# AlexanderGSC/gmres

Measured on AMD Instinct MI355X. Metric: Arnoldi iters/sec + HBM GB/s, 4096² Poisson-2D fp64, GMRES(m=95), higher is better.
Workload: dtype f64

## Files before the change

gmres_amd/_native.py:

```python
from __future__ import annotations

import ctypes
import os
import sys
import re

PKG = os.path.dirname(os.path.abspath(__file__))
LIB_DIR = os.environ.get("GK_LIB_DIR") or os.path.join(PKG, "lib")
HIP_SO = os.path.join(LIB_DIR, "libgmres_hip.so")
FHOST_SO = os.path.join(LIB_DIR, "libgmres_fhost.so")
HEADER = os.path.join(os.path.dirname(PKG), "include", "gmres_hip.h")

GK_OK = 0
GK_ERR_COMM = -6
GK_TUNE_PROJ_NT = 0
GK_TUNE_STENCIL_BLOCKS = 2
GK_TUNE_SR_BLOCKS = 28
GK_TUNE_SR_TWO_LEVEL = 29
GK_TUNE_XCHG_TIMEOUT_MS = 7
GK_TUNE_RES, GK_TUNE_RES_R2, GK_TUNE_RES_SHARE, GK_TUNE_RES_TIMEOUT_MS = 8, 9, 10, 11
GK_TUNE_VERR_ORDER = 14
GK_TUNE_HH_FUSE = 15
GK_TUNE_CHEB_STEN = 16
GK_TUNE_SPIN_WAIT = 18
GK_TUNE_GRAPH = 19
GK_TUNE_RES_QDEF = 20
GK_TUNE_RES_PC = 21
GK_TUNE_RES_FOLD = 22
GK_TUNE_RES_BLOCK = 23
GK_TUNE_WATCHDOG_MS = 24
GK_TUNE_HH_NORM_ORDER = 25
GK_TUNE_RES_PF = 27
GK_TUNE_RES_PIPE = 30
GK_TUNE_RIGHT_FUSED = 31
GK_SIDE_LEFT, GK_SIDE_RIGHT = 0, 1
GK_ERR_ARG, GK_ERR_STATE = -1, -4
GK_PREC_IDENTITY, GK_PREC_CBPR2, GK_PREC_CHEB = 0, 1, 2
(GK_KID_PROJ, GK_KID_STENCIL, GK_KID_SCALE, GK_KID_UPDATE, GK_KID_COMM, GK_KID_OTHER, GK_KID_RES, GK_KID_PREC,
 GK_KID_HALO, GK_KID_GRAPH) = range(10)
GK_KID_SR = 10
SR_PASS_NAMES = ["sr_cg_p", "sr_cg_x", "sr_cg_z", "sr_bi_p", "sr_bi_pc", "sr_bi_s", "sr_bi_sc", "sr_st1", "sr_st2",
                 "sr_bi_x", "sr_bi_pe", "sr_bi_se", "sr_dot", "sr_cg_xz", "sr_bi_pz", "sr_bi_sz"]
KID_NAMES = ["proj", "stencil", "scale", "update", "comm", "other", "res", "prec", "halo", "graph"] + SR_PASS_NAMES
GK_SR_PCG, GK_SR_BICGSTAB = 0, 1
COMM_KINDS = {0: None, 1: "rccl", 2: "local-group", 3: "xgmi-device-exchange"}
RES_VARIANTS = {0: None, 1: "prefetch", 2: "pairs", 3: "pairs+lds", 4: "w-only", 5: "w+column", 6: "blocked"}
RES_INFO_KEYS = ["variant", "G", "r2", "l2", "pf", "cw", "wo", "nt", "r2e", "l2e", "lds", "nres2", "pipe", "cheb_sten", "wt", "blk"]

c_int, c_double, c_ll, c_vp = ctypes.c_int, ctypes.c_double, ctypes.c_longlong, ctypes.c_void_p
_dp = ctypes.POINTER(ctypes.c_double)
_ip = ctypes.POINTER(ctypes.c_int)

_hip = None
_fhost = None


class GkError(RuntimeError):
    pass


def header_symbols() -> list[str]:
    txt = open(HEADER).read()
    return sorted(set(re.findall(r"^\s*(?:int|const char \*)\s*(gk_\w+)\s*\(", txt, re.M)))


_SIGS = {
    "gk_last_error": (ctypes.c_char_p, []),
    "gk_version": (c_int, []),
    "gk_runtime_info": (c_int, [_ip, _ip, _ip, ctypes.c_char_p, ctypes.c_char_p, c_int]),
    "gk_create": (c_int, [c_int, c_int, c_int, c_int, c_int, ctypes.POINTER(c_vp)]),
# ... 188 lines not shown
```

gmres_amd/csrc/gk_api.hip:

```cpp
#include <dlfcn.h>

#include <algorithm>
#include <cmath>
#include <cstdarg>
#include <cstdio>
#include <cstdlib>
#include <cstring>

#include "gk_blk.hpp"
#include "gk_host.hpp"
#include "gk_kernels.hpp"
#include "gk_resident.hpp"

using namespace gkh;
using gk::nt_auto_for;
using gk::plan_info;
using gk::plan_resident;
using gk::ResPlan;
using gk::RES_R2_BIG;

namespace gkh __attribute__((visibility("hidden"))) {

thread_local std::string g_err;

// ... 218 lines not shown

int fill_hash(gk_ctx *c, double *x, unsigned long long seed) {
    gk::k_fill_hash<<<c->nblk_stream, gk::TPB, 0, c->st>>>(x, c->nloc, c->g0, seed);
    LAUNCHCHK();
    return GK_OK;
}

int finalize(gk_ctx *c, const double *pin, int npin, double *out, int take_sqrt) {
    ProfScope ps(c, GK_KID_OTHER);
    gk::k_finalize<<<1, gk::TPB, 0, c->st>>>(pin, npin, out, take_sqrt);
    LAUNCHCHK();
    return GK_OK;
}

bool res_plan(gk_ctx *c, ResPlan &p, bool hh = false) {
    if (c->tune_res == 0 || c->res_broken || c->m > gk::RHMAX || c->res_cus <= 0 || c->res_gath == nullptr)
        return false;
    if (collective(c) && !(c->xs_on && c->nranks > 1)) return false;
    if (c->tune_res < 0 && c->res_share > 1) return false;
    const int gmax = std::max(1, std::min(gk::RGMAX, c->res_cus / std::max(1, c->res_share)));
    const int cap = c->tune_res_r2 > 0 ? c->tune_res_r2 : RES_R2_BIG;
    plan_resident(c->nloc, gmax, cap, c->tune_res_wonly, hh,
                  c->tune_nt > 0 || (c->tune_nt < 0 && c->nt_auto), p, c->tune_res_pc, c->tune_res_blk, c->tune_res_pf,
                  c->tune_res_pipe);
    if (p.wo && !hh && c->m + 1 > gk::WO_HMAX) return false;
    return true;
}

enum { RESF_CLOSE_HH = 1, RESF_UNIT_INIT = 2, RESF_PIN_LOCAL = 4 };
int res_step(gk_ctx *c, int j, const ResPlan &p, const double *pin, int npin, double *hs, double *hcopy,
             int mode = gk::RES_MGS, double *w = nullptr, i64 unit_g = -1, int flags = 0) {
    ProfScope ps(c, GK_KID_RES);
    const bool close = (flags & RESF_CLOSE_HH) && mode == gk::RES_HH_UP;
    if ((flags & ~RESF_PIN_LOCAL) != 0 && !p.wo)
        return set_err(GK_ERR_STATE, "resident flags %d need the w-only variant", flags);
    const bool pin_local = (flags & RESF_PIN_LOCAL) && mode != gk::RES_HH_DOWN && c->xs_on && c->nranks > 1;
    const int np = (mode == gk::RES_MGS ? (p.bvar >= 0 ? gk::blk_exchanges(j, p.blk) : 2 * j) : j) + (close ? 1 : 0);
    if (c->res_tag > 0xF0000000u) {
        HIPCHK(hipMemsetAsync(c->res_gath, 0, sizeof(gk::u64) * gk::RES_GATH_ALL, c->st));
        c->res_tag = 1;
    }
    gk::ResArgs a{};
    a.w = w != nullptr ? w : c->w;
    a.mode = mode;
    a.coef = mode == gk::RES_MGS ? 1.0 : 2.0;
    a.tail0 = mode == gk::RES_HH_UP ? (i64)j - c->g0 : 0;
    a.V = c->V;
// ... 1134 lines not shown
int gk_set_tuning(gk_ctx *c, int key, int value) {
    CHK(check_ctx(c));
    switch (key) {
        case GK_TUNE_PROJ_NT: c->tune_nt = value < 0 ? -1 : (value != 0); break;
        case GK_TUNE_PROJ_BLOCKS: c->tune_pj_blocks = value; break;
        case GK_TUNE_STENCIL_BLOCKS: c->tune_st_blocks = value; break;
        case GK_TUNE_CHEB_FUSED: c->tune_cheb_fused = value != 0; break;
        case GK_TUNE_XCHG_TIMEOUT_MS:
            if (value < 1) return set_err(GK_ERR_ARG, "timeout must be >= 1 ms");
            xs_set_timeout(c, value);
            break;
        case GK_TUNE_RES: c->tune_res = value < 0 ? -1 : (value != 0); break;
        case GK_TUNE_RES_R2:
            if (value != 0 && value != 2 && value != 4 && value != 8 && value != 12)
                return set_err(GK_ERR_ARG, "resident cap must be 0 (auto), 2, 4, 8 or 12");
            c->tune_res_r2 = value;
            break;
        case GK_TUNE_RES_SHARE:
            if (value < 1) return set_err(GK_ERR_ARG, "share must be >= 1");
            c->res_share = value;
            break;
        case GK_TUNE_RES_WONLY: c->tune_res_wonly = value < 0 ? -1 : (value != 0); break;
        case GK_TUNE_RES_PIPE: c->tune_res_pipe = value < 0 ? -1 : (value != 0); break;
        case GK_TUNE_HH_FUSE: c->tune_hh_fuse = value != 0; break;
        case GK_TUNE_CHEB_STEN: c->tune_cheb_sten = value != 0; break;
        case GK_TUNE_SPIN_WAIT: c->tune_spin_wait = value != 0; break;
        case GK_TUNE_GRAPH: c->tune_graph = value != 0; break;
        case GK_TUNE_RES_QDEF: c->tune_res_qdef = value < 0 ? -1 : (value != 0); break;
        case GK_TUNE_RES_PC: c->tune_res_pc = value < 0 ? -1 : (value != 0); break;
        case GK_TUNE_RES_FOLD: c->tune_res_fold = value != 0; break;
        case GK_TUNE_WATCHDOG_MS: c->watchdog_ms = std::max(0, value); break;
        case GK_TUNE_HH_NORM_ORDER: c->tune_hh_norm_order = value != 0; break;
        case GK_TUNE_RES_BLOCK:
            if (value != 1 && value != 2 && value != 4)
                return set_err(GK_ERR_ARG, "GK_TUNE_RES_BLOCK %d: blocks of 1 (strict MGS-R), 2 or 4 projections", value);
            if (c->cycle_mgs)
                c->pend_res_blk = value;
            else
                c->tune_res_blk = value;
            break;
        case GK_TUNE_SR_BLOCKS: c->tune_sr_blocks = std::max(0, value); break;
        case GK_TUNE_SR_TWO_LEVEL: c->tune_sr_two = value != 0; break;
        case GK_TUNE_RES_PF:
            if (c->cycle_mgs)
                c->pend_res_pf = value != 0;
            else
// ... 460 lines not shown
```

gmres_amd/csrc/gk_host.hpp:

```cpp
#pragma once
#include <hip/hip_runtime.h>
#include <rccl/rccl.h>

#include <condition_variable>
#include <deque>
#include <mutex>
#include <string>
#include <vector>

#include "../../include/gmres_hip.h"
#include "gk_res.hpp"

using gk::i64;

namespace gk {
struct SrDev;
struct SrMirror;
}

struct gk_group {
    int n = 0;
    std::mutex mu;
    std::condition_variable cv;
    int arrived = 0;
// ... 41 lines not shown
    i64 xs_words = 0;
    gk::XsPeers xs_peers{};
    std::vector<void *> xs_mapped;
    bool xs_ready = false, xs_on = false, xs_broken = false;
    unsigned xs_seq = 0, xs_hseq = 0;
    int *xs_err = nullptr, *xs_err_dev = nullptr;
    long long xs_tick_per_ms = 100000;
    int xs_timeout_ms = 20000;
    gk::u64 xs_timeout = 0;
    gk::u64 *res_gath = nullptr;
    double *res_gm = nullptr;
    int tune_res_blk = 1;
    int tune_res_pf = 0;
    int pend_res_blk = 0, pend_res_pf = -1;
    int watchdog_ms = 0;
    bool broken = false;
    unsigned *hold_word = nullptr, *hold_word_dev = nullptr;
    int *res_err = nullptr, *res_err_dev = nullptr;
    unsigned res_tag = 1;
    int res_cus = 0;
    int tune_res = -1;
    int tune_res_r2 = 0;
    int tune_res_pipe = -1;
    int tune_res_wonly = -1;
    int tune_verr_order = 1;
    int tune_hh_fuse = 1;
    int tune_hh_norm_order = 0;
    int res_share = 1;
    int res_timeout_ms = 20000;
    bool res_broken = false;
    gk::u64 *res_stamps = nullptr;
    bool res_split = false;
    gk::u64 *res_trace = nullptr;
    int res_trace_j = 0, res_trace_mode = -1;
    int res_trace_g = 0, res_trace_np = 0;
    int vec = 2, JT = 16;
    dim3 sgrid;
    int sr_JT = 64, tune_sr_blocks = 0;
    int tune_sr_two = 1;
    bool sr_two = false;
    dim3 sr_sgrid;
    int np_sr = 0;
    int np_st = 0, np_pj = 0, nblk_stream = 0;
    int last_np = 0;
    int tune_cheb_fused = 1;
    int tune_cheb_sten = 1;
// ... 103 lines not shown
```

gmres_amd/csrc/gk_res.hpp:

```cpp
#pragma once
#include "gk_common.hpp"
#include "gk_cheb.hpp"

namespace gk {

constexpr int XS_MAXR = 16;
constexpr int XS_MAXV = 128;
constexpr i64 XS_RED_WORDS = 2LL * XS_MAXR * XS_MAXV * 2;
typedef unsigned long long u64;
struct XsPeers {
    u64 *p[XS_MAXR];
};
enum { XS_SLAB = 0, XS_VEC = 1, XS_BCAST = 2 };

__device__ __forceinline__ void xs_put(u64 *q, unsigned seq, unsigned data) {
    __hip_atomic_store(q, ((u64)seq << 32) | data, __ATOMIC_RELAXED, __HIP_MEMORY_SCOPE_SYSTEM);
}

__device__ __forceinline__ int xs_flag(const int *err) {
    return __hip_atomic_load(err, __ATOMIC_RELAXED, __HIP_MEMORY_SCOPE_SYSTEM);
}

enum { XG_ABORT = -1, XG_LATE = 0, XG_OK = 1 };
__device__ __forceinline__ int xs_get(const u64 *q, unsigned seq, u64 deadline, unsigned *data, const int *err) {
// ... 174 lines not shown
    for (int q = 0; q < a.nranks; ++q) {
        const unsigned lo = __shfl(d, 2 * q, 64), hi = __shfl(d, 2 * q + 1, 64);
        const double v = __longlong_as_double((long long)(((u64)hi << 32) | lo));
        r = (q == 0) ? v : r + v;
    }
    return r;
}

__device__ __forceinline__ bool res_pin_fold(const ResArgs &a, double &h, double *bc, int *okf) {
    if (!a.pin_local) return true;
    if (threadIdx.x < 64) {
        bool ok = true;
        const double r = res_rank_sum(a, -1, h, ok);
        if (threadIdx.x == 0) {
            bc[0] = r;
            *okf = ok ? 1 : 0;
        }
    }
    __syncthreads();
    h = bc[0];
    return *okf != 0;
}

template <int NW = RWAVES, bool TR = false, int SLEEP = RES_POLL_SLEEP>
__device__ __forceinline__ void res_exchange(const ResArgs &a, int p, const double *sm, double *bc, int *okf) {
    const int lane = threadIdx.x;
    const int G = gridDim.x;
    const unsigned tag = a.tag0 + (unsigned)p;
    auto rep_slot = [&](int r) -> u64 * {
        return a.gath + (RES_NREP > 1 ? RES_REP0 + r * RES_REP_STRIDE : 0) + (i64)(p & 1) * G * 2;
    };
    u64 *slot = rep_slot((int)(blockIdx.x % RES_NREP));
    double s = sm[0];
#pragma unroll
    for (int w = 1; w < NW; ++w) s += sm[w];
    u64 t_pub = 0;
    if (TR && a.trace != nullptr) t_pub = wall_clock64();
    if (RES_PUSHERS > 1 && res_pusher(a)) asm volatile("s_waitcnt vmcnt(0)" ::: "memory");
    if (lane < 2 * RES_NREP) {
        const u64 bits = (u64)__double_as_longlong(s);
        const int half = lane & 1;
        __hip_atomic_store(rep_slot(lane >> 1) + 2 * blockIdx.x + half,
                           ((u64)tag << 32) | (half ? (unsigned)(bits >> 32) : (unsigned)bits), __ATOMIC_RELAXED,
                           __HIP_MEMORY_SCOPE_AGENT);
    }
    const u64 deadline = wall_clock64() + a.timeout;
    double acc = 0.0;
    bool all_ok = true;
    if (a.nranks == 1 || blockIdx.x < RES_PUSHERS) {
        for (int c0 = 0; c0 < 2 * G && all_ok; c0 += 512) {
            unsigned v[8];
            for (;;) {
                u64 x[8];
#pragma unroll
                for (int k = 0; k < 8; ++k) {
                    const int g = c0 + lane + 64 * k;
                    x[k] = __hip_atomic_load(slot + (g < 2 * G ? g : 0), __ATOMIC_RELAXED, __HIP_MEMORY_SCOPE_AGENT);
                }
                bool ok = true;
#pragma unroll
                for (int k = 0; k < 8; ++k) {
                    const bool in = c0 + lane + 64 * k < 2 * G;
                    v[k] = in ? (unsigned)x[k] : 0u;
                    ok = ok && (!in || (unsigned)(x[k] >> 32) == tag);
                }
                if (__all(ok)) break;
                if (wall_clock64() > deadline) {
                    all_ok = false;
// ... 119 lines not shown
```

gmres_amd/csrc/gk_resident.hip:

```cpp
#include <hip/hip_runtime.h>

#include <algorithm>
#include <atomic>
#include <cstdarg>
#include <cstdio>

#include "../../include/gmres_hip.h"
#include "gk_blk.hpp"
#include "gk_res.hpp"
#include "gk_resident.hpp"

namespace gk {

template <int R2, int L2, bool PF, bool NT, bool CW, int MODE>
__global__ __launch_bounds__(RT, 2) void k_mgs_res(ResArgs a) {
    extern __shared__ double2 lw[];
    __shared__ double sm[RWAVES];
    __shared__ double bc[1];
    __shared__ int okf;
    __shared__ double hsh[RHMAX + 1];
    constexpr int RB = PF ? R2 : 1;
    constexpr int DT = CW ? RT - 64 : RT;
    const int t = threadIdx.x;
    const bool data = !CW || t >= 64;
// ... 264 lines not shown
#define GK_RES_TOUCH 24
#endif
constexpr int TOUCH = GK_RES_TOUCH;
#ifndef GK_RES_TOUCH_MGS
#define GK_RES_TOUCH_MGS 28
#endif
constexpr int TOUCH_MGS = GK_RES_TOUCH_MGS;
#ifndef GK_RES_TOUCH_MGS_PIPE
#define GK_RES_TOUCH_MGS_PIPE 20
#endif
constexpr int TOUCH_MGS_PIPE = GK_RES_TOUCH_MGS_PIPE;
#ifndef GK_RES_TOUCH_PACE
#define GK_RES_TOUCH_PACE 24
#endif
constexpr int TOUCH_PACE = GK_RES_TOUCH_PACE;
#ifndef GK_RES_TOUCH_PACE_HH
#define GK_RES_TOUCH_PACE_HH 0
#endif
constexpr int TOUCH_PACE_HH = GK_RES_TOUCH_PACE_HH;
#ifndef GK_RES_PIPE_D
#define GK_RES_PIPE_D 8
#endif
constexpr int PIPE_D = GK_RES_PIPE_D;

template <class F, int... I>
__device__ __forceinline__ void seq_apply(F &&f, std::integer_sequence<int, I...>) {
    (f(std::integral_constant<int, I>{}), ...);
}
template <int N, class F>
__device__ __forceinline__ void seq_for(F &&f) {
    seq_apply(f, std::make_integer_sequence<int, N>{});
}

template <int RW, int LW, int MODE, int WBT = WB, bool PIPE = false>
__global__ __launch_bounds__(WT, 1) void k_mgs_wres(ResArgs a) {
    extern __shared__ double2 lw[];
    __shared__ double sm[WT / 64];
    __shared__ double bc[1];
    __shared__ int okf;
    __shared__ int xdone;
    __shared__ double hsh[MODE == RES_MGS ? WO_HMAX : 1];
    const int t = threadIdx.x;
    constexpr int mode = MODE;
    constexpr int PACE = MODE == RES_MGS ? TOUCH_PACE : TOUCH_PACE_HH;
    constexpr int TCH = MODE == RES_MGS ? (PIPE ? TOUCH_MGS_PIPE : TOUCH_MGS) : TOUCH;
    const int j = a.j, np = res_np(mode, j);
    const i64 n2 = a.n >> 1, ld2 = a.ld >> 1;
    const i64 nch = a.nres2 / WT;
    const i64 bq = blockIdx.x;
    const i64 c0 = bq * a.r2e, cend = c0 + a.r2e < nch ? c0 + a.r2e : nch;
    const i64 l0 = (i64)gridDim.x * a.r2e + bq * a.l2e, lend = l0 + a.l2e < nch ? l0 + a.l2e : nch;
    const i64 tail0 = mode == RES_HH_UP ? a.tail0 : 0;
    const double2 *__restrict__ V2 = reinterpret_cast<const double2 *>(a.V);
    double2 *__restrict__ W2 = reinterpret_cast<double2 *>(a.w);
    ResClock clk;
    clk.start(a.stamps);
    int touch_sink = 0;
    const i64 sstride = (i64)gridDim.x * WT;
    const i64 sbase = a.nres2 + (i64)res_stream_wg() * WT + t;
    double2 wr[RW];
    if (mode == RES_HH_DOWN && a.unit_init) {
        const i64 u = a.unit_e;
        auto unit2 = [&](i64 e2) { return double2{2 * e2 == u ? 1.0 : 0.0, 2 * e2 + 1 == u ? 1.0 : 0.0}; };
#pragma unroll
        for (int k = 0; k < RW; ++k) wr[k] = (c0 + k < cend) ? unit2((c0 + k) * WT + t) : double2{0.0, 0.0};
        for (int k = 0; k < LW; ++k)
            if (l0 + k < lend) lw[k * WT + t] = unit2((l0 + k) * WT + t);
        for (i64 e = sbase; e < n2; e += sstride) W2[e] = unit2(e);
        if ((a.n & 1) && blockIdx.x == gridDim.x - 1 && t == 0) a.w[a.n - 1] = (a.n - 1 == u) ? 1.0 : 0.0;
    } else {
#pragma unroll
        for (int k = 0; k < RW; ++k) wr[k] = (PIPE || c0 + k < cend) ? W2[(c0 + k) * WT + t] : double2{0.0, 0.0};
        for (int k = 0; k < LW; ++k)
            if (PIPE || l0 + k < lend) lw[k * WT + t] = W2[(l0 + k) * WT + t];
    }
    auto red = [&](double &acc, const double2 &v, const double2 &b, int kind, i64 e2, bool chk) {
        if (kind == RK_DOT) {
            acc = acc + v.x * b.x;
            acc = acc + v.y * b.y;
        } else if (kind == RK_NORM) {
            sq_acc(acc, v, e2, tail0, chk);
        }
    };
    const i64 wc0 = c0, wl0 = l0;
    auto pass = [&](double ch, int i, int q, int kind) -> double {
        const double2 *__restrict__ A2 = V2 + (i64)i * ld2;
        const double2 *__restrict__ B2 = V2 + (i64)q * ld2;
        const bool dot = kind == RK_DOT;
        double acc = 0.0;
        i64 c0 = wc0, l0 = wl0;
        if constexpr (PIPE) {
            int zero = 0;
            asm volatile("" : "+s"(zero));
            c0 += zero;
            l0 += zero;
        }
        if constexpr (PIPE) {
            constexpr int D = WBT, NCH = RW + LW;
            static_assert(MODE == RES_MGS && NCH > D && 2 * (D - 1) <= 63,
                          "pipelined pass: the MGS step, counts within vmcnt's 6 bits, V_q default policy");
            d2v pa[D], pb[D];
            const unsigned lo = (unsigned)t * (unsigned)sizeof(double2);
            const double2 *Ar = A2 + c0 * WT, *Al = A2 + l0 * WT, *Br = B2 + c0 * WT, *Bl = B2 + l0 * WT;
            __builtin_amdgcn_s_waitcnt(0x0f70);
            auto held = [&](int k) { return k < RW ? c0 + k < cend : l0 + (k - RW) < lend; };
            auto issue = [&](auto kc) {
                constexpr int k = decltype(kc)::value;
                const double2 *ap = k < RW ? Ar + k * WT : Al + (k - RW) * WT;
                const double2 *bq = k < RW ? Br + k * WT : Bl + (k - RW) * WT;
                const double2 *bp = dot ? bq : Ar;
                d2v &da = pa[k % D], &db = pb[k % D];
                const unsigned off = lo;
                asm volatile("global_load_dwordx4 %0, %1, %2 nt" : "=v"(da) : "v"(off), "s"(ap));
                asm volatile("global_load_dwordx4 %0, %1, %2" : "=v"(db) : "v"(off), "s"(bp));
            };
            auto wait = [&](auto kc) {
                constexpr int k = decltype(kc)::value;
                constexpr int younger = NCH - 1 - k < D - 1 ? NCH - 1 - k : D - 1;
                d2v &da = pa[k % D], &db = pb[k % D];
                asm volatile("s_waitcnt vmcnt(%2)" : "+v"(da), "+v"(db) : "i"(2 * younger));
            };
            auto consume = [&](auto kc) {
                constexpr int k = decltype(kc)::value;
                const double2 av{pa[k % D].x, pa[k % D].y}, bv{pb[k % D].x, pb[k % D].y};
                if (!held(k)) return;
                if constexpr (k < RW) {
                    wr[k].x = wr[k].x - ch * av.x;
                    wr[k].y = wr[k].y - ch * av.y;
                    red(acc, wr[k], bv, kind, (c0 + k) * WT + t, false);
                } else {
                    constexpr int kl = k - RW;
                    double2 wv = lw[kl * WT + t];
                    wv.x = wv.x - ch * av.x;
                    wv.y = wv.y - ch * av.y;
                    lw[kl * WT + t] = wv;
                    red(acc, wv, bv, kind, (l0 + kl) * WT + t, false);
                }
            };
            seq_for<D>(issue);
            seq_for<NCH>([&](auto kc) {
                constexpr int k = decltype(kc)::value;
                wait(kc);
                consume(kc);
                if constexpr (k + D < NCH) issue(std::integral_constant<int, k + D>{});
            });
            return acc;
        }
        auto rbatch = [&](const int k0) {
            double2 av[WBT], bv[WBT];
#pragma unroll
            for (int u = 0; u < WBT; ++u) {
                const i64 c = c0 + k0 + u;
                if (k0 + u < RW && c < cend) {
                    av[u] = ldv<true>(A2 + c * WT + t);
                    if (dot) bv[u] = ldv<false>(B2 + c * WT + t);
                }
            }
#pragma unroll
            for (int u = 0; u < WBT; ++u) {
                const int k = k0 + u;
                if (k < RW && c0 + k < cend) {
                    wr[k].x = wr[k].x - ch * av[u].x;
// ... 38 lines not shown
                    if (dot) bv[u] = ldv<false>(B2 + e);
                }
            }
#pragma unroll
            for (int u = 0; u < 2; ++u) {
                const i64 e = e0 + u * sstride;
                if (e < n2) {
                    wv[u].x = wv[u].x - ch * av[u].x;
                    wv[u].y = wv[u].y - ch * av[u].y;
                    W2[e] = wv[u];
                    red(acc, wv[u], bv[u], kind, e, mode == RES_HH_UP && 2 * a.nres2 < tail0);
                }
            }
        }
        if ((a.n & 1) && blockIdx.x == gridDim.x - 1 && t == 0) {
            const i64 e = a.n - 1;
            const double x = a.w[e] - ch * a.V[(i64)i * a.ld + e];
            a.w[e] = x;
            if (kind == RK_DOT) acc = acc + x * a.V[(i64)q * a.ld + e];
            if (kind == RK_NORM && e >= tail0) acc = acc + x * x;
        }
        return acc;
    };
    int xi = 0;
    auto reduce = [&](double acc, double &h, int touch_col) -> bool {
        clk.passed(a.stamps);
        acc = wave_sum(acc);
        if ((t & 63) == 0) sm[t >> 6] = acc;
        if (PACE > 0 && t == 0) xdone = 0;
        __syncthreads();
        if (t < 64) {
            res_exchange<WT / 64, MODE == RES_MGS, RES_POLL_SLEEP>(a, xi, sm, bc, &okf);
            if (PACE > 0 && t == 0) *(volatile int *)&xdone = 1;
        } else if constexpr (TCH > 0) {
            if (touch_col >= 0) {
                const i64 r0 = c0, r1 = cend;
                const i64 lines = (i64)32 * (r1 - r0 < TCH ? (r1 - r0 > 0 ? r1 - r0 : 0) : TCH);
                const char *base = reinterpret_cast<const char *>(V2 + (i64)touch_col * ld2 + r0 * WT);
                for (i64 l = t - 64; l < lines; l += WT - 64) {
                    if constexpr (PACE > 0) {
                        if (*(volatile int *)&xdone) break;
                    }
                    const char *ptr = base + l * 128;
                    asm volatile("global_load_dword %0, %1, off" : "+v"(touch_sink) : "v"(ptr) : "memory");
                    if constexpr (PACE > 0) __builtin_amdgcn_s_sleep(PACE);
                }
            }
        }
        __syncthreads();
        if constexpr (TCH > 0) asm volatile("s_waitcnt vmcnt(0)" : : "v"(touch_sink) : "memory");
        ++xi;
        h = bc[0];
        clk.waited(a.stamps);
        return okf != 0;
    };
    auto kind_of = [&](int p) { return p < np - 1 ? RK_DOT : (mode == RES_MGS ? RK_NORM : RK_NONE); };
    double h;
    bool ok = true;
    if (mode == RES_HH_DOWN) {
        const int q = res_col(mode, j, 0);
        double acc = 0.0;
        if (a.unit_known) {
            if (blockIdx.x == 0 && t == 0 && a.unit_e >= 0) acc = a.V[(i64)q * a.ld + a.unit_e];
        } else {
            acc = pass(0.0, q, q, RK_DOT);
        }
        ok = reduce(acc, h, kind_of(0) == RK_DOT ? res_col(mode, j, 1) : -1);
    } else {
        double s = 0.0;
        for (int k = t; k < a.npin; k += WT) s += a.pin[k];
        s = wave_sum(s);
        if ((t & 63) == 0) sm[t >> 6] = s;
        __syncthreads();
        h = sm[0];
#pragma unroll
        for (int w = 1; w < WT / 64; ++w) h += sm[w];
        __syncthreads();
        ok = res_pin_fold(a, h, bc, &okf);
    }
    for (int p = 0; p < np && ok; ++p) {
        const int i = res_col(mode, j, p);
        const int kind = kind_of(p);
        if (mode == RES_MGS && blockIdx.x == 0 && t == 0) hsh[i] = (p < j ? 0.0 : hsh[i]) + h;
        const double acc = pass(mode == RES_MGS ? h : a.coef * h, i, res_col(mode, j, p + 1), kind);
        if (kind != RK_NONE)
            ok = reduce(acc, h, p + 1 < np && kind_of(p + 1) == RK_DOT ? res_col(mode, j, p + 2) : -1);
    }
    if (!ok) return;
    const bool close = mode == RES_HH_UP && a.close_hh;
    if (mode != RES_MGS) {
        double acc = 0.0;
        const bool up = mode == RES_HH_UP;
#pragma unroll
        for (int k = 0; k < RW; ++k)
            if (c0 + k < cend) {
                if (!close) W2[(c0 + k) * WT + t] = wr[k];
                if (up) sq_acc(acc, wr[k], (c0 + k) * WT + t, tail0, c0 + k == 0);
            }
        for (int k = 0; k < LW; ++k)
            if (l0 + k < lend) {
                const double2 v = lw[k * WT + t];
                if (!close) W2[(l0 + k) * WT + t] = v;
                if (up) sq_acc(acc, v, (l0 + k) * WT + t, tail0, l0 + k == 0);
            }
        if (up) {
            for (i64 e = sbase; e < n2; e += sstride) sq_acc(acc, W2[e], e, tail0, 2 * e < tail0 + 2);
            if ((a.n & 1) && blockIdx.x == gridDim.x - 1 && t == 0 && a.n - 1 >= tail0) {
                const double x = a.w[a.n - 1];
                acc = acc + x * x;
// ... 332 lines not shown
    if (RES_PCS && n2 <= (i64)G * RES_PCS_RW * RES_PC_NT) return 8 * n2;
    const int rx = hh ? RES_PC_RX : RES_PC_RX_MGS;
    const i64 cap = (i64)G * RES_PC_RW * RES_PC_NT, cached = (i64)G * (rx + RES_PC_LX) * RES_PC_NT;
    const i64 r = std::min(n2, cap), c = std::min(r, cached);
    return 8 * c + 16 * (r - c) + 32 * (n2 - r);
}

i64 pairs_bytes(i64 n2, int G) {
    const i64 rp = (i64)G * RES_R2_BIG * gk::RT, lp = (i64)G * RES_L2 * gk::RT;
    auto clamp = [](i64 v) { return v < 0 ? (i64)0 : v; };
    const i64 pr = std::min(n2, rp), pl = std::min(clamp(n2 - rp), lp), ps = clamp(n2 - rp - lp);
    return 8 * pr + 16 * pl + 32 * ps;
}

i64 wonly_bytes(i64 n2, int G) {
    const i64 rw = (i64)G * (RES_RW + RES_LW) * gk::WT;
    const i64 wr = std::min(n2, rw), ws = n2 > rw ? n2 - rw : 0;
    return 16 * wr + 32 * ws;
}

static bool wonly_pays(i64 n2, int G) { return wonly_bytes(n2, G) < pairs_bytes(n2, G); }

void plan_resident(i64 nloc, int gmax, int cap, int tune_wonly, bool hh, bool nt, ResPlan &p,
                   int tune_pc, int tune_blk, int tune_pf, int tune_pipe) {
    const i64 n2 = nloc / 2;
    const i64 dcw = gk::RT - 64;
    const int gcw = (int)std::max<i64>(1, std::min<i64>(gmax, (n2 + 2 * dcw - 1) / (2 * dcw)));
    const i64 need = (n2 + (i64)gcw * dcw - 1) / ((i64)gcw * dcw);
    p = ResPlan{};
    static const int pfs[] = {2, 4, 8};
    for (int s : pfs)
        if (s <= cap && (p.r2 == 0 || p.r2 < need)) p.r2 = s;
    auto spread = [&](i64 dt, int rmax, int lmax) {
        const i64 nchf = n2 / dt, G = p.G;
        p.r2e = (int)std::min<i64>(rmax, (nchf + G - 1) / G);
        const i64 rest = std::max<i64>(0, nchf - G * p.r2e);
        p.l2e = (int)std::min<i64>(lmax, (rest + G - 1) / G);
        p.nres2 = std::min<i64>(nchf, G * (p.r2e + p.l2e)) * dt;
    };
    const int var = gk::blk_variant((n2 + (i64)gmax * 512 - 1) / ((i64)gmax * 512));
    const bool pf = !hh && tune_blk == 1 && var != gk::BLK_WONLY && tune_pf > 0;
    if (!hh && (tune_blk > 1 || pf)) {
        p.G = gmax;
        const gk::BlkGeom g = gk::blk_geom(var, tune_blk);
        p.blk = tune_blk;
        p.bvar = var;
        p.wt = g.nt;
// ... 12 lines not shown
        p.pf = p.cw = true;
        spread(dcw, p.r2, 0);
    } else if (tune_wonly <= 0 && (tune_pc > 0 ? pc_fits : (tune_pc < 0 && pc_pays))) {
        p.G = gmax;
        p.pc = true;
        p.wt = RES_PC_NT;
        spread(RES_PC_NT, RES_PC_RW, 0);
        p.pcs = RES_PCS && p.r2e <= RES_PCS_RW;
        p.r2 = p.pcs ? RES_PCS_RX : (hh ? RES_PC_RX : RES_PC_RX_MGS);
        p.l2 = p.pcs ? RES_PCS_LX : RES_PC_LX;
        p.lds = p.l2 * RES_PC_NT * (int)sizeof(double2);
        p.nt = true;
        return;
    } else if (tune_wonly > 0 || (tune_wonly < 0 && wonly_pays(n2, gmax))) {
        p.G = gmax;
        p.wo = true;
        p.wt = gk::WT;
        p.r2 = 0;
        spread(gk::WT, hh ? RES_RW_HH : RES_RW, hh ? RES_LW_HH : RES_LW);
        p.lds = (hh ? RES_LW_HH : RES_LW) * gk::WT * (int)sizeof(double2);
        p.nt = true;
        p.pipe = RES_PIPE_OK && !hh && (tune_pipe < 0 ? RES_PIPE : tune_pipe != 0) && p.r2e == RES_RW &&
                 p.l2e == RES_LW && nloc % 2 == 0 && n2 == (i64)p.G * (RES_RW + RES_LW) * gk::WT && p.nres2 == n2;
        return;
    } else {
        p.G = gmax;
        p.r2 = RES_R2_BIG;
        const i64 dt = gk::RT, regs = (i64)p.G * RES_R2_BIG * dt;
        p.l2 = n2 / dt * dt > regs ? RES_L2 : 0;
        spread(dt, RES_R2_BIG, p.l2);
    }
    p.lds = std::max<int>(RES_LDS_MIN, p.l2 * (p.cw ? gk::RT - 64 : gk::RT) * (int)sizeof(double2));
    p.wt = gk::RT;
    p.nt = nt;
}

bool nt_auto_for(i64 max_nloc) { return max_nloc * 8 > (i64)48 * 1024 * 1024; }

void plan_info(const ResPlan &p, bool on, long long *info) {
    for (int k = 0; k < GK_RES_INFO_LEN; ++k) info[k] = 0;
    if (!on) return;
    info[RPI_VARIANT] = p.bvar >= 0 ? GK_RES_BLOCKED
                        : p.pc    ? GK_RES_WCOL
                                  : (p.wo ? GK_RES_WONLY
                                          : (p.pf ? GK_RES_PREFETCH : (p.l2 > 0 ? GK_RES_PAIRS_LDS : GK_RES_PAIRS)));
    info[RPI_BLK] = p.bvar >= 0 ? p.blk : 1;
    info[RPI_G] = p.G;
    info[RPI_R2] = p.r2;
    info[RPI_L2] = p.l2;
    info[RPI_PF] = p.pf;
    info[RPI_CW] = p.cw;
    info[RPI_WO] = p.wo;
    info[RPI_NT] = p.nt;
    info[RPI_R2E] = p.r2e;
    info[RPI_L2E] = p.l2e;
    info[RPI_LDS] = p.lds;
    info[RPI_NRES2] = p.nres2;
    info[RPI_WT] = p.wt;
    info[RPI_PIPE] = p.pipe;
}

namespace {

int fail(std::string &msg, int code, const char *fmt, ...) {
    char buf[512];
    va_list ap;
    va_start(ap, fmt);
    vsnprintf(buf, sizeof buf, fmt, ap);
    va_end(ap);
    msg = buf;
    return code;
}

int dyn_lds(const void *kernel, int dev, int lds, std::atomic<int> *memo, std::string &msg) {
    if (dev < 0 || dev >= ATTR_DEVS) return fail(msg, GK_ERR_ARG, "device id %d out of range", dev);
    const hipError_t e = ensure_dyn_lds(kernel, dev, lds, memo);
    if (e != hipSuccess)
        return fail(msg, GK_ERR_HIP, "%s:%d hipFuncSetAttribute(dynamic LDS %d): %s", __FILE__, __LINE__, lds,
                    hipGetErrorString(e));
    return GK_OK;
}

// ... 1 lines not shown
    const hipError_t e = hipGetLastError();
    if (e != hipSuccess) return fail(msg, GK_ERR_HIP, "resident step launch: %s", hipGetErrorString(e));
    return GK_OK;
}

template <int R2, int L2, bool PF, bool NT, bool CW, int MODE>
int launch_res_m(const ResPlan &p, const ResArgs &a, int dev, hipStream_t st, std::string &msg) {
    static std::atomic<int> attr[ATTR_DEVS];
    const int e = dyn_lds(reinterpret_cast<const void *>(&k_mgs_res<R2, L2, PF, NT, CW, MODE>), dev, p.lds, attr, msg);
    if (e != GK_OK) return e;
    k_mgs_res<R2, L2, PF, NT, CW, MODE><<<p.G, RT, p.lds, st>>>(a);
    return launched(msg);
}

template <int R2, int L2, bool PF, bool NT, bool CW>
int launch_res_t(const ResPlan &p, const ResArgs &a, int dev, hipStream_t st, std::string &msg) {
    switch (a.mode) {
        case RES_HH_UP: return launch_res_m<R2, L2, PF, NT, CW, RES_HH_UP>(p, a, dev, st, msg);
        case RES_HH_DOWN: return launch_res_m<R2, L2, PF, NT, CW, RES_HH_DOWN>(p, a, dev, st, msg);
        default: return launch_res_m<R2, L2, PF, NT, CW, RES_MGS>(p, a, dev, st, msg);
    }
}

template <int MODE, bool PIPE = false>
int launch_wres_m(const ResPlan &p, const ResArgs &a, int dev, hipStream_t st, std::string &msg) {
    constexpr int RW = MODE == RES_MGS ? RES_RW : RES_RW_HH;
    constexpr int LW = MODE == RES_MGS ? RES_LW : RES_LW_HH;
    constexpr int WBT = PIPE ? PIPE_D : (MODE == RES_MGS ? WB : WB_HH);
    static std::atomic<int> attr[ATTR_DEVS];
    const int e = dyn_lds(reinterpret_cast<const void *>(&k_mgs_wres<RW, LW, MODE, WBT, PIPE>), dev, p.lds, attr, msg);
    if (e != GK_OK) return e;
    k_mgs_wres<RW, LW, MODE, WBT, PIPE><<<p.G, WT, p.lds, st>>>(a);
    return launched(msg);
}

int launch_wres(const ResPlan &p, const ResArgs &a, int dev, hipStream_t st, std::string &msg) {
    switch (a.mode) {
        case RES_HH_UP: return launch_wres_m<RES_HH_UP>(p, a, dev, st, msg);
        case RES_HH_DOWN: return launch_wres_m<RES_HH_DOWN>(p, a, dev, st, msg);
        default:
            if constexpr (RES_PIPE_OK) {
                if (p.pipe) {
                    if (p.r2e != RES_RW || p.l2e != RES_LW || (a.n & 1) || a.nres2 != a.n / 2)
                        return fail(msg, GK_ERR_STATE, "pipelined w-only step on a plan that is not full (%d + %d chunks)",
                                    p.r2e, p.l2e);
                    return launch_wres_m<RES_MGS, true>(p, a, dev, st, msg);
                }
            }
            return launch_wres_m<RES_MGS>(p, a, dev, st, msg);
    }
}

template <int RW, int RX, int LX, int MODE>
int launch_wpc_k(const ResPlan &p, const ResArgs &a, int dev, hipStream_t st, std::string &msg) {
    constexpr int WBT = MODE == RES_MGS ? RES_PC_WB : RES_PC_WB_HH;
    static std::atomic<int> attr[ATTR_DEVS];
    if (p.r2e > RW || p.lds < LX * RES_PC_NT * (int)sizeof(double2))
        return fail(msg, GK_ERR_STATE, "column-cache plan (%d chunks, %d B LDS) does not fit k_mgs_wpc<%d,%d,%d>", p.r2e,
                    p.lds, RW, RX, LX);
    const int e = dyn_lds(reinterpret_cast<const void *>(&k_mgs_wpc<RW, RX, LX, MODE, WBT, RES_PC_NT>), dev,
                          p.lds, attr, msg);
    if (e != GK_OK) return e;
    k_mgs_wpc<RW, RX, LX, MODE, WBT, RES_PC_NT><<<p.G, RES_PC_NT, p.lds, st>>>(a);
    return launched(msg);
}

template <int MODE>
int launch_wpc_m(const ResPlan &p, const ResArgs &a, int dev, hipStream_t st, std::string &msg) {
// ... 40 lines not shown
```

gmres_amd/csrc/gk_resident.hpp:

```cpp
#pragma once
#include <string>

#include "gk_common.hpp"

namespace gk {

struct ResArgs;

constexpr int RES_R2_BIG = 12;

struct ResPlan {
    int G = 0, r2 = 0, l2 = 0;
    int r2e = 0, l2e = 0;
    bool pf = false, nt = false, cw = false, wo = false;
    bool pc = false;
    bool pcs = false;
    int blk = 0;
    int bvar = -1;
    int wt = 0;
    bool pipe = false;
    i64 nres2 = 0;
    int lds = 0;
};

GK_HIDDEN i64 pc_bytes(i64 n2, int G, bool hh);
GK_HIDDEN i64 pairs_bytes(i64 n2, int G);
GK_HIDDEN i64 wonly_bytes(i64 n2, int G);

GK_HIDDEN void plan_resident(i64 nloc, int gmax, int cap, int tune_wonly, bool hh, bool nt, ResPlan &p,
                             int tune_pc = -1, int tune_blk = 1, int tune_pf = 0, int tune_pipe = -1);
GK_HIDDEN bool nt_auto_for(i64 max_nloc);

enum { RPI_VARIANT = 0, RPI_G, RPI_R2, RPI_L2, RPI_PF, RPI_CW, RPI_WO, RPI_NT, RPI_R2E, RPI_L2E, RPI_LDS, RPI_NRES2, RPI_PIPE,
       RPI_CHEB_STEN, RPI_WT, RPI_BLK };
GK_HIDDEN void plan_info(const ResPlan &p, bool on, long long *info);

GK_HIDDEN int res_launch(const ResPlan &p, const ResArgs &a, int dev, hipStream_t st, std::string &msg);

}
```

include/gmres_hip.h:

```cpp
#ifndef GMRES_HIP_H
#define GMRES_HIP_H

#ifdef __cplusplus
extern "C" {
#endif

#define GK_OK 0
#define GK_ERR_ARG (-1)
#define GK_ERR_HIP (-2)
#define GK_ERR_RCCL (-3)
#define GK_ERR_STATE (-4)
#define GK_ERR_NOMEM (-5)
#define GK_ERR_COMM (-6)

#define GK_PREC_IDENTITY 0
#define GK_PREC_CBPR2 1
#define GK_PREC_CHEB 2

#define GK_KID_PROJ 0
#define GK_KID_STENCIL 1
#define GK_KID_SCALE 2
#define GK_KID_UPDATE 3
#define GK_KID_COMM 4
#define GK_KID_OTHER 5
// ... 79 lines not shown
#define GK_SR_BICGSTAB 1
int gk_sr_start(gk_ctx *ctx, int solver, double tol, int max_iter);
int gk_sr_iterate(gk_ctx *ctx, int k);
int gk_sr_status(gk_ctx *ctx, int wait, int *executed, int *done, double *res);
int gk_sr_history(gk_ctx *ctx, double *hist, int n);

int gk_profile_enable(gk_ctx *ctx, int enable);
int gk_profile_reset(gk_ctx *ctx);
int gk_profile_read(gk_ctx *ctx, int kid, double *total_ms, long long *launches);
int gk_profile_res_split(gk_ctx *ctx, int mode, int which, double *pass_ms, double *wait_ms, double *total_ms,
                         long long *launches);
int gk_profile_res_wg(gk_ctx *ctx, int which, double *pass_ms, double *wait_ms, int maxwg, int *nwg);
int gk_profile_res_trace(gk_ctx *ctx, int arm, int j, int mode, unsigned long long *out, int maxwg, int maxx,
                         int *nwg, int *nx, double *tick_per_ms);
int gk_sync(gk_ctx *ctx);

#define GK_RES_NONE 0
#define GK_RES_PREFETCH 1
#define GK_RES_PAIRS 2
#define GK_RES_PAIRS_LDS 3
#define GK_RES_WONLY 4
#define GK_RES_WCOL 5
#define GK_RES_BLOCKED 6
#define GK_RES_INFO_LEN 16
int gk_res_plan_query(long long nloc, int cus, int share, int hh, int nt, int block, long long *info);
int gk_res_info(gk_ctx *ctx, int hh, long long *info);

#define GK_TUNE_PROJ_NT 0
#define GK_TUNE_PROJ_BLOCKS 1
#define GK_TUNE_STENCIL_BLOCKS 2
#define GK_TUNE_CHEB_FUSED 6
#define GK_TUNE_XCHG_TIMEOUT_MS 7
#define GK_TUNE_RES 8
#define GK_TUNE_RES_R2 9
#define GK_TUNE_RES_SHARE 10
#define GK_TUNE_RES_TIMEOUT_MS 11
#define GK_TUNE_RES_WONLY 13
#define GK_TUNE_VERR_ORDER 14
#define GK_TUNE_HH_FUSE 15
#define GK_TUNE_CHEB_STEN 16
#define GK_TUNE_SPIN_WAIT 18
#define GK_TUNE_GRAPH 19
#define GK_TUNE_RES_QDEF 20
#define GK_TUNE_RES_PC 21
#define GK_TUNE_RES_FOLD 22
#define GK_TUNE_RES_BLOCK 23
#define GK_TUNE_WATCHDOG_MS 24
#define GK_TUNE_HH_NORM_ORDER 25
#define GK_TUNE_RES_PF 27
#define GK_TUNE_SR_BLOCKS 28
#define GK_TUNE_SR_TWO_LEVEL 29
#define GK_TUNE_RES_PIPE 30
#define GK_TUNE_RIGHT_FUSED 31
int gk_set_tuning(gk_ctx *ctx, int key, int value);
int gk_debug_hold_stream(gk_ctx *ctx, int hold);

int gk_poisson5(int nside, int nlines, const double *x, const double *halo_lo,
                const double *halo_hi, double *y, void *stream);
int gk_precond_apply(int nside, int kind, const double *params, int degree, const double *r,
                     double *z, double *scratch, void *stream);
int gk_mgs_project(long long n, double *w, const double *va, double *result, void *stream);
int gk_dot(long long n, const double *a, const double *b, double *result, void *stream);

#ifdef __cplusplus
}
#endif
#endif
```

Measured before the change: 263.0.

## Prefetch next pass's ring head into registers during the resident reduction exchange

In the pipelined resident MGS kernel, the first CARRY chunks of the next projection pass's column pair are loaded into registers while the grid-wide reduction exchange is in flight. Wave 0 issues them after publishing its partial, and the other waves issue them alongside the cache touch. The pipelined pass then skips issuing those chunks. The aim is to hide HBM latency behind the exchange wait. The cost is more VGPR pressure, a different touch depth, and a mode that is disabled for multi-rank runs.

```diff
diff --git a/gmres_amd/_native.py b/gmres_amd/_native.py
--- a/gmres_amd/_native.py
+++ b/gmres_amd/_native.py
@@ -33,6 +33,7 @@
 GK_TUNE_RES_PF = 27
 GK_TUNE_RES_PIPE = 30
 GK_TUNE_RIGHT_FUSED = 31
+GK_TUNE_RES_PIPE_CARRY = 32
 GK_SIDE_LEFT, GK_SIDE_RIGHT = 0, 1
 GK_ERR_ARG, GK_ERR_STATE = -1, -4
 GK_PREC_IDENTITY, GK_PREC_CBPR2, GK_PREC_CHEB = 0, 1, 2
@@ -45,7 +46,8 @@
 GK_SR_PCG, GK_SR_BICGSTAB = 0, 1
 COMM_KINDS = {0: None, 1: "rccl", 2: "local-group", 3: "xgmi-device-exchange"}
 RES_VARIANTS = {0: None, 1: "prefetch", 2: "pairs", 3: "pairs+lds", 4: "w-only", 5: "w+column", 6: "blocked"}
-RES_INFO_KEYS = ["variant", "G", "r2", "l2", "pf", "cw", "wo", "nt", "r2e", "l2e", "lds", "nres2", "pipe", "cheb_sten", "wt", "blk"]
+RES_INFO_KEYS = ["variant", "G", "r2", "l2", "pf", "cw", "wo", "nt", "r2e", "l2e", "lds", "nres2", "pipe", "cheb_sten", "wt", "blk",
+                 "carry"]
 
 c_int, c_double, c_ll, c_vp = ctypes.c_int, ctypes.c_double, ctypes.c_longlong, ctypes.c_void_p
 _dp = ctypes.POINTER(ctypes.c_double)
diff --git a/gmres_amd/csrc/gk_api.hip b/gmres_amd/csrc/gk_api.hip
--- a/gmres_amd/csrc/gk_api.hip
+++ b/gmres_amd/csrc/gk_api.hip
@@ -264,7 +264,8 @@
     const int cap = c->tune_res_r2 > 0 ? c->tune_res_r2 : RES_R2_BIG;
     plan_resident(c->nloc, gmax, cap, c->tune_res_wonly, hh,
                   c->tune_nt > 0 || (c->tune_nt < 0 && c->nt_auto), p, c->tune_res_pc, c->tune_res_blk, c->tune_res_pf,
-                  c->tune_res_pipe);
+                  c->tune_res_pipe, c->tune_res_carry);
+    if (c->nranks > 1) p.carry = 0;
     if (p.wo && !hh && c->m + 1 > gk::WO_HMAX) return false;
     return true;
 }
@@ -1445,6 +1446,7 @@
             break;
         case GK_TUNE_RES_WONLY: c->tune_res_wonly = value < 0 ? -1 : (value != 0); break;
         case GK_TUNE_RES_PIPE: c->tune_res_pipe = value < 0 ? -1 : (value != 0); break;
+        case GK_TUNE_RES_PIPE_CARRY: c->tune_res_carry = value < 0 ? -1 : (value != 0); break;
         case GK_TUNE_HH_FUSE: c->tune_hh_fuse = value != 0; break;
         case GK_TUNE_CHEB_STEN: c->tune_cheb_sten = value != 0; break;
         case GK_TUNE_SPIN_WAIT: c->tune_spin_wait = value != 0; break;
diff --git a/gmres_amd/csrc/gk_host.hpp b/gmres_amd/csrc/gk_host.hpp
--- a/gmres_amd/csrc/gk_host.hpp
+++ b/gmres_amd/csrc/gk_host.hpp
@@ -87,6 +87,7 @@
     int tune_res = -1;
     int tune_res_r2 = 0;
     int tune_res_pipe = -1;
+    int tune_res_carry = -1;
     int tune_res_wonly = -1;
     int tune_verr_order = 1;
     int tune_hh_fuse = 1;
diff --git a/gmres_amd/csrc/gk_res.hpp b/gmres_amd/csrc/gk_res.hpp
--- a/gmres_amd/csrc/gk_res.hpp
+++ b/gmres_amd/csrc/gk_res.hpp
@@ -220,8 +220,12 @@
     return *okf != 0;
 }
 
-template <int NW = RWAVES, bool TR = false, int SLEEP = RES_POLL_SLEEP>
-__device__ __forceinline__ void res_exchange(const ResArgs &a, int p, const double *sm, double *bc, int *okf) {
+struct ResNoHook {
+    __device__ __forceinline__ void operator()() const {}
+};
+template <int NW = RWAVES, bool TR = false, int SLEEP = RES_POLL_SLEEP, class HOOK = ResNoHook>
+__device__ __forceinline__ void res_exchange(const ResArgs &a, int p, const double *sm, double *bc, int *okf,
+                                             HOOK &&published = HOOK{}) {
     const int lane = threadIdx.x;
     const int G = gridDim.x;
     const unsigned tag = a.tag0 + (unsigned)p;
@@ -242,6 +246,7 @@
                            ((u64)tag << 32) | (half ? (unsigned)(bits >> 32) : (unsigned)bits), __ATOMIC_RELAXED,
                            __HIP_MEMORY_SCOPE_AGENT);
     }
+    published();
     const u64 deadline = wall_clock64() + a.timeout;
     double acc = 0.0;
     bool all_ok = true;
diff --git a/gmres_amd/csrc/gk_resident.hip b/gmres_amd/csrc/gk_resident.hip
--- a/gmres_amd/csrc/gk_resident.hip
+++ b/gmres_amd/csrc/gk_resident.hip
@@ -310,6 +310,15 @@
 #define GK_RES_PIPE_D 8
 #endif
 constexpr int PIPE_D = GK_RES_PIPE_D;
+#ifndef GK_RES_PIPE_CARRY
+#define GK_RES_PIPE_CARRY 7
+#endif
+constexpr int PIPE_CARRY = GK_RES_PIPE_CARRY;
+static_assert(PIPE_CARRY >= 0 && PIPE_CARRY <= PIPE_D, "GK_RES_PIPE_CARRY: 0 .. GK_RES_PIPE_D chunks of the ring");
+#ifndef GK_RES_TOUCH_MGS_CARRY
+#define GK_RES_TOUCH_MGS_CARRY 20
+#endif
+constexpr int TOUCH_MGS_CARRY = GK_RES_TOUCH_MGS_CARRY;
 
 template <class F, int... I>
 __device__ __forceinline__ void seq_apply(F &&f, std::integer_sequence<int, I...>) {
@@ -320,8 +329,10 @@
     seq_apply(f, std::make_integer_sequence<int, N>{});
 }
 
-template <int RW, int LW, int MODE, int WBT = WB, bool PIPE = false>
+template <int RW, int LW, int MODE, int WBT = WB, bool PIPE = false, int CARRY = 0>
 __global__ __launch_bounds__(WT, 1) void k_mgs_wres(ResArgs a) {
+    static_assert(CARRY >= 0 && CARRY <= WBT && (CARRY == 0 || (PIPE && MODE == RES_MGS && CARRY <= RW)),
+                  "carried chunks: a head of the pipelined pass's ring, register chunks of the MGS step");
     extern __shared__ double2 lw[];
     __shared__ double sm[WT / 64];
     __shared__ double bc[1];
@@ -331,7 +342,7 @@
     const int t = threadIdx.x;
     constexpr int mode = MODE;
     constexpr int PACE = MODE == RES_MGS ? TOUCH_PACE : TOUCH_PACE_HH;
-    constexpr int TCH = MODE == RES_MGS ? (PIPE ? TOUCH_MGS_PIPE : TOUCH_MGS) : TOUCH;
+    constexpr int TCH = MODE == RES_MGS ? (PIPE ? (CARRY > 0 ? TOUCH_MGS_CARRY : TOUCH_MGS_PIPE) : TOUCH_MGS) : TOUCH;
     const int j = a.j, np = res_np(mode, j);
     const i64 n2 = a.n >> 1, ld2 = a.ld >> 1;
     const i64 nch = a.nres2 / WT;
@@ -347,6 +358,7 @@
     const i64 sstride = (i64)gridDim.x * WT;
     const i64 sbase = a.nres2 + (i64)res_stream_wg() * WT + t;
     double2 wr[RW];
+    [[maybe_unused]] d2v ra[CARRY > 0 ? WBT : 1], rb[CARRY > 0 ? WBT : 1];
     if (mode == RES_HH_DOWN && a.unit_init) {
         const i64 u = a.unit_e;
         auto unit2 = [&](i64 e2) { return double2{2 * e2 == u ? 1.0 : 0.0, 2 * e2 + 1 == u ? 1.0 : 0.0}; };
@@ -387,7 +399,13 @@
             constexpr int D = WBT, NCH = RW + LW;
             static_assert(MODE == RES_MGS && NCH > D && 2 * (D - 1) <= 63,
                           "pipelined pass: the MGS step, counts within vmcnt's 6 bits, V_q default policy");
-            d2v pa[D], pb[D];
+            [[maybe_unused]] d2v pl[CARRY > 0 ? 1 : D], ql[CARRY > 0 ? 1 : D];
+            auto &pa = *[&]() {
+                if constexpr (CARRY > 0) return &ra; else return &pl;
+            }();
+            auto &pb = *[&]() {
+                if constexpr (CARRY > 0) return &rb; else return &ql;
+            }();
             const unsigned lo = (unsigned)t * (unsigned)sizeof(double2);
             const double2 *Ar = A2 + c0 * WT, *Al = A2 + l0 * WT, *Br = B2 + c0 * WT, *Bl = B2 + l0 * WT;
             __builtin_amdgcn_s_waitcnt(0x0f70);
@@ -425,7 +443,7 @@
                     red(acc, wv, bv, kind, (l0 + kl) * WT + t, false);
                 }
             };
-            seq_for<D>(issue);
+            seq_for<D - CARRY>([&](auto kc) { issue(std::integral_constant<int, decltype(kc)::value + CARRY>{}); });
             seq_for<NCH>([&](auto kc) {
                 constexpr int k = decltype(kc)::value;
                 wait(kc);
@@ -510,19 +528,53 @@
         }
         return acc;
     };
+    [[maybe_unused]] auto head = [&](int pn) {
+        int zero = 0;
+        asm volatile("" : "+s"(zero));
+        const double2 *Ar = V2 + (i64)res_col(mode, j, pn) * ld2 + (wc0 + zero) * WT;
+        const double2 *Br = V2 + (i64)res_col(mode, j, pn + 1) * ld2 + (wc0 + zero) * WT;
+        const bool dot = pn < np - 1;
+        const unsigned lo = (unsigned)t * (unsigned)sizeof(double2);
+        seq_for<CARRY>([&](auto kc) {
+            constexpr int k = decltype(kc)::value;
+            const double2 *ap = Ar + k * WT;
+            const double2 *bp = dot ? Br + k * WT : Ar;
+            d2v &da = ra[k], &db = rb[k];
+            const unsigned off = lo;
+            asm volatile("global_load_dwordx4 %0, %1, %2 nt" : "=v"(da) : "v"(off), "s"(ap));
+            asm volatile("global_load_dwordx4 %0, %1, %2" : "=v"(db) : "v"(off), "s"(bp));
+        });
+    };
+    [[maybe_unused]] auto head_landed = [&]() {
+        asm volatile("s_waitcnt vmcnt(0)" ::: "memory");
+        seq_for<CARRY>([&](auto kc) {
+            constexpr int k = decltype(kc)::value;
+            d2v &da = ra[k], &db = rb[k];
+            asm volatile("" : "+v"(da), "+v"(db));
+        });
+    };
     int xi = 0;
-    auto reduce = [&](double acc, double &h, int touch_col) -> bool {
+    auto reduce = [&](double acc, double &h, int touch_col, [[maybe_unused]] int head_p = 0) -> bool {
         clk.passed(a.stamps);
         acc = wave_sum(acc);
         if ((t & 63) == 0) sm[t >> 6] = acc;
         if (PACE > 0 && t == 0) xdone = 0;
         __syncthreads();
         if (t < 64) {
-            res_exchange<WT / 64, MODE == RES_MGS, RES_POLL_SLEEP>(a, xi, sm, bc, &okf);
+            if constexpr (CARRY > 0) {
+                asm volatile("; gk-audit: arm wave0");
+                res_exchange<WT / 64, MODE == RES_MGS, RES_POLL_SLEEP>(a, xi, sm, bc, &okf, [&]() { head(head_p); });
+            } else {
+                res_exchange<WT / 64, MODE == RES_MGS, RES_POLL_SLEEP>(a, xi, sm, bc, &okf);
+            }
             if (PACE > 0 && t == 0) *(volatile int *)&xdone = 1;
-        } else if constexpr (TCH > 0) {
-            if (touch_col >= 0) {
-                const i64 r0 = c0, r1 = cend;
+        } else {
+            if constexpr (CARRY > 0) {
+                asm volatile("; gk-audit: arm waves123");
+                head(head_p);
+            }
+            if (TCH > 0 && touch_col >= 0) {
+                const i64 r0 = c0 + CARRY, r1 = cend;
                 const i64 lines = (i64)32 * (r1 - r0 < TCH ? (r1 - r0 > 0 ? r1 - r0 : 0) : TCH);
                 const char *base = reinterpret_cast<const char *>(V2 + (i64)touch_col * ld2 + r0 * WT);
                 for (i64 l = t - 64; l < lines; l += WT - 64) {
@@ -536,7 +588,9 @@
             }
         }
         __syncthreads();
+        if constexpr (CARRY > 0) asm volatile("; gk-audit: arms end");
         if constexpr (TCH > 0) asm volatile("s_waitcnt vmcnt(0)" : : "v"(touch_sink) : "memory");
+        if constexpr (CARRY > 0) head_landed();
         ++xi;
         h = bc[0];
         clk.waited(a.stamps);
@@ -566,13 +620,17 @@
         __syncthreads();
         ok = res_pin_fold(a, h, bc, &okf);
     }
+    if constexpr (CARRY > 0) {
+        head(0);
+        head_landed();
+    }
     for (int p = 0; p < np && ok; ++p) {
         const int i = res_col(mode, j, p);
         const int kind = kind_of(p);
         if (mode == RES_MGS && blockIdx.x == 0 && t == 0) hsh[i] = (p < j ? 0.0 : hsh[i]) + h;
         const double acc = pass(mode == RES_MGS ? h : a.coef * h, i, res_col(mode, j, p + 1), kind);
         if (kind != RK_NONE)
-            ok = reduce(acc, h, p + 1 < np && kind_of(p + 1) == RK_DOT ? res_col(mode, j, p + 2) : -1);
+            ok = reduce(acc, h, p + 1 < np && kind_of(p + 1) == RK_DOT ? res_col(mode, j, p + 2) : -1, p + 1);
     }
     if (!ok) return;
     const bool close = mode == RES_HH_UP && a.close_hh;
@@ -951,7 +1009,7 @@
 static bool wonly_pays(i64 n2, int G) { return wonly_bytes(n2, G) < pairs_bytes(n2, G); }
 
 void plan_resident(i64 nloc, int gmax, int cap, int tune_wonly, bool hh, bool nt, ResPlan &p,
-                   int tune_pc, int tune_blk, int tune_pf, int tune_pipe) {
+                   int tune_pc, int tune_blk, int tune_pf, int tune_pipe, int tune_carry) {
     const i64 n2 = nloc / 2;
     const i64 dcw = gk::RT - 64;
     const int gcw = (int)std::max<i64>(1, std::min<i64>(gmax, (n2 + 2 * dcw - 1) / (2 * dcw)));
@@ -1010,6 +1068,7 @@
         p.nt = true;
         p.pipe = RES_PIPE_OK && !hh && (tune_pipe < 0 ? RES_PIPE : tune_pipe != 0) && p.r2e == RES_RW &&
                  p.l2e == RES_LW && nloc % 2 == 0 && n2 == (i64)p.G * (RES_RW + RES_LW) * gk::WT && p.nres2 == n2;
+        p.carry = p.pipe && (tune_carry < 0 || tune_carry != 0) ? gk::PIPE_CARRY : 0;
         return;
     } else {
         p.G = gmax;
@@ -1046,6 +1105,7 @@
     info[RPI_NRES2] = p.nres2;
     info[RPI_WT] = p.wt;
     info[RPI_PIPE] = p.pipe;
+    info[RPI_CARRY] = p.carry;
 }
 
 namespace {
@@ -1093,15 +1153,16 @@
     }
 }
 
-template <int MODE, bool PIPE = false>
+template <int MODE, bool PIPE = false, int CARRY = 0>
 int launch_wres_m(const ResPlan &p, const ResArgs &a, int dev, hipStream_t st, std::string &msg) {
     constexpr int RW = MODE == RES_MGS ? RES_RW : RES_RW_HH;
     constexpr int LW = MODE == RES_MGS ? RES_LW : RES_LW_HH;
     constexpr int WBT = PIPE ? PIPE_D : (MODE == RES_MGS ? WB : WB_HH);
     static std::atomic<int> attr[ATTR_DEVS];
-    const int e = dyn_lds(reinterpret_cast<const void *>(&k_mgs_wres<RW, LW, MODE, WBT, PIPE>), dev, p.lds, attr, msg);
+    const int e =
+        dyn_lds(reinterpret_cast<const void *>(&k_mgs_wres<RW, LW, MODE, WBT, PIPE, CARRY>), dev, p.lds, attr, msg);
     if (e != GK_OK) return e;
-    k_mgs_wres<RW, LW, MODE, WBT, PIPE><<<p.G, WT, p.lds, st>>>(a);
+    k_mgs_wres<RW, LW, MODE, WBT, PIPE, CARRY><<<p.G, WT, p.lds, st>>>(a);
     return launched(msg);
 }
 
@@ -1115,6 +1176,13 @@
                     if (p.r2e != RES_RW || p.l2e != RES_LW || (a.n & 1) || a.nres2 != a.n / 2)
                         return fail(msg, GK_ERR_STATE, "pipelined w-only step on a plan that is not full (%d + %d chunks)",
                                     p.r2e, p.l2e);
+                    if constexpr (PIPE_CARRY > 0) {
+                        if (p.carry != 0) {
+                            if (a.nranks != 1 || p.carry != PIPE_CARRY)
+                                return fail(msg, GK_ERR_STATE, "carried pass (%d chunks) on %d ranks", p.carry, a.nranks);
+                            return launch_wres_m<RES_MGS, true, PIPE_CARRY>(p, a, dev, st, msg);
+                        }
+                    }
                     return launch_wres_m<RES_MGS, true>(p, a, dev, st, msg);
                 }
             }
diff --git a/gmres_amd/csrc/gk_resident.hpp b/gmres_amd/csrc/gk_resident.hpp
--- a/gmres_amd/csrc/gk_resident.hpp
+++ b/gmres_amd/csrc/gk_resident.hpp
@@ -19,6 +19,7 @@
     int bvar = -1;
     int wt = 0;
     bool pipe = false;
+    int carry = 0;
     i64 nres2 = 0;
     int lds = 0;
 };
@@ -28,11 +29,12 @@
 GK_HIDDEN i64 wonly_bytes(i64 n2, int G);
 
 GK_HIDDEN void plan_resident(i64 nloc, int gmax, int cap, int tune_wonly, bool hh, bool nt, ResPlan &p,
-                             int tune_pc = -1, int tune_blk = 1, int tune_pf = 0, int tune_pipe = -1);
+                             int tune_pc = -1, int tune_blk = 1, int tune_pf = 0, int tune_pipe = -1,
+                             int tune_carry = -1);
 GK_HIDDEN bool nt_auto_for(i64 max_nloc);
 
 enum { RPI_VARIANT = 0, RPI_G, RPI_R2, RPI_L2, RPI_PF, RPI_CW, RPI_WO, RPI_NT, RPI_R2E, RPI_L2E, RPI_LDS, RPI_NRES2, RPI_PIPE,
-       RPI_CHEB_STEN, RPI_WT, RPI_BLK };
+       RPI_CHEB_STEN, RPI_WT, RPI_BLK, RPI_CARRY };
 GK_HIDDEN void plan_info(const ResPlan &p, bool on, long long *info);
 
 GK_HIDDEN int res_launch(const ResPlan &p, const ResArgs &a, int dev, hipStream_t st, std::string &msg);
diff --git a/include/gmres_hip.h b/include/gmres_hip.h
--- a/include/gmres_hip.h
+++ b/include/gmres_hip.h
@@ -125,7 +125,7 @@
 #define GK_RES_WONLY 4
 #define GK_RES_WCOL 5
 #define GK_RES_BLOCKED 6
-#define GK_RES_INFO_LEN 16
+#define GK_RES_INFO_LEN 17
 int gk_res_plan_query(long long nloc, int cus, int share, int hh, int nt, int block, long long *info);
 int gk_res_info(gk_ctx *ctx, int hh, long long *info);
 
@@ -155,6 +155,7 @@
 #define GK_TUNE_SR_TWO_LEVEL 29
 #define GK_TUNE_RES_PIPE 30
 #define GK_TUNE_RIGHT_FUSED 31
+#define GK_TUNE_RES_PIPE_CARRY 32
 int gk_set_tuning(gk_ctx *ctx, int key, int value);
 int gk_debug_hold_stream(gk_ctx *ctx, int hold);
 
```

After: 273.5, median of 6. 4.0% higher.
